# franioli/icepy4d

Measured on AMD Instinct MI355X. Metric: matched stereo image-pairs/sec (4096 kpts, 1080p), higher is better.
Workload: dtype f32

## Files before the change

icepy4d_amd/csrc/attention_bx.hip:

```cpp
#include "bf16x3.h"
#include "common.h"
#include "kernels.h"
#include "sp_post.h"

#include <cstdlib>

namespace im {

static constexpr int BKT = 32;
static constexpr int BKS = 144;
static constexpr int BVS = 192;
static constexpr int BK_PLANE = BKT * BKS, BV_PLANE = BKT * BVS;
static constexpr int B_STAGE = 3 * BK_PLANE + 3 * BV_PLANE;
static constexpr int B_LDS = 2 * B_STAGE;
static constexpr int DPL = BKT * 128;
static constexpr int D_LDS = 3 * 3 * (DPL + DPL);

__device__ __forceinline__ f32x16 mfma_attn(u32x4 a, u32x4 b, f32x16 c) {
#ifdef BX_ABL_NO_MFMA
    c[0] += __uint_as_float(a.x ^ b.x);
    return c;
#else
    return mfma_bf(a, b, c);
#endif
}

__device__ __forceinline__ void stage4(unsigned char* plane0, int plane_bytes, int off, float4 x) {
    unsigned h0, m0, l0, h1, m1, l1;
    split2(x.x, x.y, h0, m0, l0);
    split2(x.z, x.w, h1, m1, l1);
    *reinterpret_cast<u32x2*>(plane0 + off) = u32x2{h0, h1};
    *reinterpret_cast<u32x2*>(plane0 + plane_bytes + off) = u32x2{m0, m1};
    *reinterpret_cast<u32x2*>(plane0 + 2 * plane_bytes + off) = u32x2{l0, l1};
}

typedef __attribute__((address_space(3))) bf16x4 lds_bf16x4;
__device__ __forceinline__ u32x2 tr_read(const unsigned char* p) {
#ifdef BX_ABL_NO_VREAD
    const unsigned x = (unsigned)(unsigned long long)p;
    return u32x2{x, 0x3f803f80u};
#else
    const bf16x4 v = __builtin_amdgcn_ds_read_tr16_b64_v4bf16((lds_bf16x4*)(p));
    return __builtin_bit_cast(u32x2, v);
#endif
}
__device__ __forceinline__ u32x4 kf_read(const unsigned char* p) {
#ifdef BX_ABL_NO_KREAD
    const unsigned x = (unsigned)(unsigned long long)p;
    return u32x4{x, 0x3f803f80u, x, 0x3f803f80u};
#else
    return *reinterpret_cast<const u32x4*>(p);
#endif
}

static constexpr float BX_SLACK = 8.f;
__device__ __forceinline__ float bmax3(float a, float b, float c) { return __builtin_fmaxf(__builtin_fmaxf(a, b), c); }

template <bool TAIL>
__device__ __forceinline__ float softmax_ref(f32x16& s, int kb, int nk, int hh, float& m_run, float& l_run, f32x16& o0, f32x16& o1) {
    if (TAIL) {
#pragma unroll
        for (int r = 0; r < 16; ++r)
            if (kb + acc_row(r, hh) >= nk) s[r] = -INFINITY;
    }
    float mx0 = bmax3(s[0], s[1], s[2]), mx1 = bmax3(s[3], s[4], s[5]);
    mx0 = bmax3(mx0, s[6], s[7]); mx1 = bmax3(mx1, s[8], s[9]);
    mx0 = bmax3(mx0, s[10], s[11]); mx1 = bmax3(mx1, s[12], s[13]);
    float mx = bmax3(mx0, mx1, fmaxf(s[14], s[15]));
    mx = fmaxf(mx, __shfl_xor(mx, 32));
    if (__builtin_amdgcn_ballot_w64(mx > m_run + BX_SLACK) != 0) {
        asm volatile("" ::: "memory");
        const float m_new = fmaxf(m_run, mx);
        const float alpha = __builtin_amdgcn_exp2f(m_run - m_new);
        l_run *= alpha;
        o0 *= alpha;
        o1 *= alpha;
        m_run = m_new;
    }
    return (TAIL && m_run == -INFINITY) ? 0.f : m_run;
}
__device__ __forceinline__ void softmax_exp(f32x16& s, float m_use, float& l_run) {
    float r0 = 0.f, r1 = 0.f;
#pragma unroll
    for (int r = 0; r < 16; r += 2) {
        s[r] = __builtin_amdgcn_exp2f(s[r] - m_use);
        s[r + 1] = __builtin_amdgcn_exp2f(s[r + 1] - m_use);
        r0 += s[r]; r1 += s[r + 1];
    }
    float rs = r0 + r1;
    rs += __shfl_xor(rs, 32);
    l_run += rs;
}

__global__ __launch_bounds__(256) void kv_planes_kernel(AttnArgs a) {
    const long rid = (long)blockIdx.x * 32 + (threadIdx.x >> 3);
    const int d8 = threadIdx.x & 7;
    const long per_image = (long)a.heads * a.n_max;
    if (rid >= per_image * a.batch) return;
    const int z = (int)(rid / per_image), rem = (int)(rid - (long)z * per_image), head = rem / a.n_max, row = rem - head * a.n_max;
    if (a.active && a.active[(z >> 1) * a.pstride] == 0) return;
    const int n = a.n_ptr ? a.n_ptr[(z >> 1) * a.pstride + (z & 1)] : a.n_max;
    if (row >= n) return;
    const float* src = (blockIdx.y ? a.v : a.k) + (long)z * a.bstride + (long)head * a.hstride + (long)row * 64 + d8 * 8;
    const float4 u = *reinterpret_cast<const float4*>(src), w = *reinterpret_cast<const float4*>(src + 4);
    const Planes p = split8(u.x, u.y, u.z, u.w, w.x, w.y, w.z, w.w);
    unsigned char* dst = reinterpret_cast<unsigned char*>(a.planes) + ((long)blockIdx.y * per_image * a.batch + rid) * 384 + d8 * 16;
    *reinterpret_cast<u32x4*>(dst) = p.h;
    *reinterpret_cast<u32x4*>(dst + 128) = p.m;
    *reinterpret_cast<u32x4*>(dst + 256) = p.l;
}

template <bool PRE, bool DMA>
__global__ __launch_bounds__(256, 2) void flash_attn_bx_kernel(AttnArgs a) {
    static_assert(PRE || !DMA, "the DMA form stages planes");
    extern __shared__ __attribute__((aligned(16))) unsigned char bsm[];
    constexpr int RD = DMA ? 3 : 2;
    constexpr int KS = DMA ? 128 : BKS, VS = DMA ? 128 : BVS;
    constexpr int KPL = BKT * KS, VPL = BKT * VS;

    const int gsz = (a.batch % 2 == 0) ? 2 : a.batch;
    const int hz = a.heads * gsz;
    const int nqb = (a.n_max + 127) / 128;
    const int per_group = hz * nqb * (a.part ? ATTN_MAX_SPLIT : 1);
    const int grp_idx = blockIdx.x / per_group;
    const int bid = blockIdx.x - grp_idx * per_group;
    const int head = (bid % hz) % a.heads, z = grp_idx * gsz + (bid % hz) / a.heads;
    const int y = a.cross ? (z ^ 1) : z;
    if (a.active && a.active[(z >> 1) * a.pstride] == 0) return;
    const int nq = a.n_ptr ? a.n_ptr[(z >> 1) * a.pstride + (z & 1)] : a.n_max;
    const int nk_all = a.n_ptr ? a.n_ptr[(y >> 1) * a.pstride + (y & 1)] : a.n_max;
    const int qblk = (bid / hz) % nqb, split = (bid / hz) / nqb;
    const int qb = qblk * 128;
    if (qb >= nq || nk_all <= 0) return;
    int n_split = 1, k0 = 0, nk = nk_all;
    if (a.part) {
        const int steps_all = (nk_all + BKT - 1) / BKT;
        const int want = nq > 2048 ? 1 : (nq > 1024 ? 2 : ATTN_MAX_SPLIT);
        const int steps_per = (steps_all + want - 1) / want;
        n_split = (steps_all + steps_per - 1) / steps_per;
        k0 = split * steps_per * BKT;
        nk = min(nk_all - k0, steps_per * BKT);
    }
    if (split >= n_split) return;

    const int tid = threadIdx.x, lane = tid & 63, wave = tid >> 6;
    const int c = lane & 31, hh = lane >> 5;
    const int qrow = qb + wave * 32 + c;

    const float* Q = a.q + (long)z * a.bstride + (long)head * a.hstride;
    __amdgpu_buffer_rsrc_t K, V;
    u32x4 Kd = {}, Vd = {};
    if constexpr (PRE) {
        const long rows = (long)a.heads * a.n_max * a.batch;
        const unsigned char* kp = reinterpret_cast<const unsigned char*>(a.planes) + (((long)y * a.heads + head) * a.n_max + k0) * 384;
        K = make_rsrc(kp, nk * 384);
        V = make_rsrc(kp + rows * 384, nk * 384);
        if constexpr (DMA) { Kd = make_rsrc4(kp, nk * 384); Vd = make_rsrc4(kp + rows * 384, nk * 384); }
    } else {
        K = make_rsrc(a.k + (long)y * a.bstride + (long)head * a.hstride + (long)k0 * 64, nk * 256);
        V = make_rsrc(a.v + (long)y * a.bstride + (long)head * a.hstride + (long)k0 * 64, nk * 256);
    }

    u32x4 qh[4], qm[4], ql[4];
    {
        const float* qp = Q + (long)min(qrow, nq - 1) * 64 + hh * 8;
        const float c2 = a.scale * 1.4426950408889634f;
#pragma unroll
        for (int s = 0; s < 4; ++s) {
            const float4 u = *reinterpret_cast<const float4*>(qp + 16 * s), w = *reinterpret_cast<const float4*>(qp + 16 * s + 4);
            const Planes p = split8(u.x * c2, u.y * c2, u.z * c2, u.w * c2, w.x * c2, w.y * c2, w.z * c2, w.w * c2);
            qh[s] = p.h; qm[s] = p.m; ql[s] = p.l;
        }
    }

    f32x16 o0, o1;
#pragma unroll
    for (int r = 0; r < 16; ++r) { o0[r] = 0.f; o1[r] = 0.f; }
    float m_run = -INFINITY, l_run = 0.f;
    const int nt = (nk + BKT - 1) / BKT;

    unsigned char* const kring = bsm;
    unsigned char* const vring = bsm + RD * 3 * KPL;
    int kq[4], dv[2];
    const int vq = (lane & 15) >> 2;
    if constexpr (DMA) {
#pragma unroll
        for (int s4 = 0; s4 < 4; ++s4) kq[s4] = c * 128 + (((2 * s4 + hh) ^ ((c >> 1) & 7)) << 4);
        const int base = (4 * hh + vq) * 128 + (((lane >> 4) & 1) * 2 + ((lane & 3) >> 1)) * 16 + (lane & 1) * 8, sv = (vq >> 1) & 1;
        dv[0] = base + sv * 64; dv[1] = base + (1 - sv) * 64;
    } else {
#pragma unroll
        for (int s4 = 0; s4 < 4; ++s4) kq[s4] = c * BKS + hh * 16 + 32 * s4;
        const int base = (4 * hh + vq) * BVS + ((lane >> 4) & 1) * 32 + (lane & 3) * 8;
        dv[0] = base; dv[1] = base + 64;
    }

    u32x4 pk[3], pv[3];
    float4 fk[2], fv[2];
    int lk[3], lv[3];
    if constexpr (PRE) {
#pragma unroll
        for (int i = 0; i < 3; ++i) {
            const int id = tid + 256 * i, row = id / 24, rem = id - 24 * row;
            lk[i] = (rem >> 3) * BK_PLANE + row * BKS + (rem & 7) * 16;
            lv[i] = (rem >> 3) * BV_PLANE + row * BVS + (rem & 7) * 16;
        }
    }
    const unsigned voff = PRE ? tid * 16u : ((tid >> 4) * 64 + (tid & 15) * 4) * 4u;
    const int st_k = (tid >> 4) * BKS + (tid & 15) * 8, st_v = (tid >> 4) * BVS + (tid & 15) * 8;
    auto load_k = [&](int tile) {
        if constexpr (PRE) {
            const unsigned so = (unsigned)tile * (BKT * 384u);
#pragma unroll
            for (int i = 0; i < 3; ++i) pk[i] = __builtin_amdgcn_raw_buffer_load_b128(K, voff, so + 4096u * i, 0);
        } else {
            const unsigned so = (unsigned)tile * (BKT * 256u);
// ... 275 lines not shown
        if (threadIdx.x == 0) {
            unsigned long long* cp = a.clock + 2 * (blockIdx.x % CLOCK_PROBE_SLOTS);
            cp[0] = ck1 - ck0; cp[1] = cr1 - cr0;
        }
    }
    {
        const int t = nt - 1;
        m_use = softmax_ref<true>(sc, t * BKT, nk, hh, m_run, l_run, o0, o1);
        softmax_exp(sc, m_use, l_run);
        pv_mul(r0, sc);
    }

    if (n_split > 1) {
        const long prow = (((long)z * a.heads + head) * a.n_max + min(qrow, a.n_max - 1)) * 66;
        const long pstride = (long)a.batch * a.heads * a.n_max * 66;
        float* pp = a.part + (long)split * pstride + prow;
        if (qrow < nq) {
#pragma unroll
            for (int g = 0; g < 4; ++g) {
                *reinterpret_cast<float2*>(pp + 8 * g + 4 * hh) = make_float2(o0[4 * g], o0[4 * g + 1]);
                *reinterpret_cast<float2*>(pp + 8 * g + 4 * hh + 2) = make_float2(o0[4 * g + 2], o0[4 * g + 3]);
                *reinterpret_cast<float2*>(pp + 32 + 8 * g + 4 * hh) = make_float2(o1[4 * g], o1[4 * g + 1]);
                *reinterpret_cast<float2*>(pp + 32 + 8 * g + 4 * hh + 2) = make_float2(o1[4 * g + 2], o1[4 * g + 3]);
            }
            if (hh == 0) { pp[64] = m_run; pp[65] = l_run; }
        }
        __threadfence();
        __syncthreads();
        int* flag = reinterpret_cast<int*>(bsm);
        if (tid == 0) {
            int* cnt = a.counters + ((long)z * a.heads + head) * nqb + qblk;
            const int old = atomicAdd(cnt, 1);
            *flag = (old == n_split - 1);
            if (old == n_split - 1) *cnt = 0;
        }
        __syncthreads();
        if (!*flag) return;
        __threadfence();
        float m = -INFINITY;
        for (int sidx = 0; sidx < n_split; ++sidx) m = fmaxf(m, a.part[(long)sidx * pstride + prow + 64]);
        l_run = 0.f;
#pragma unroll
        for (int r = 0; r < 16; ++r) { o0[r] = 0.f; o1[r] = 0.f; }
        for (int sidx = 0; sidx < n_split; ++sidx) {
            const float* ps = a.part + (long)sidx * pstride + prow;
            const float w = __builtin_amdgcn_exp2f(ps[64] - m);
            l_run += w * ps[65];
#pragma unroll
            for (int g = 0; g < 4; ++g)
#pragma unroll
                for (int q = 0; q < 4; ++q) {
                    o0[4 * g + q] += w * ps[8 * g + 4 * hh + q];
                    o1[4 * g + q] += w * ps[32 + 8 * g + 4 * hh + q];
                }
        }
    }

    if (qrow < nq) {
        const float inv = 1.f / l_run;
        float* op = a.out + (long)z * a.out_bstride + (long)qrow * a.ldo + head * 64;
#pragma unroll
        for (int g = 0; g < 4; ++g) {
            const float4 w0 = make_float4(o0[4 * g] * inv, o0[4 * g + 1] * inv, o0[4 * g + 2] * inv, o0[4 * g + 3] * inv);
            const float4 w1 = make_float4(o1[4 * g] * inv, o1[4 * g + 1] * inv, o1[4 * g + 2] * inv, o1[4 * g + 3] * inv);
            *reinterpret_cast<float4*>(op + 8 * g + 4 * hh) = w0;
            *reinterpret_cast<float4*>(op + 32 + 8 * g + 4 * hh) = w1;
        }
    }
}

hipError_t launch_attn_planes(const AttnArgs& a, hipStream_t s) {
    static const bool f32_form = [] { const char* e = getenv("IM_ATTN_F32"); return e && atoi(e) != 0; }();
    if (!a.planes || a.n_max <= 0 || f32_form || a.f32_form) return hipSuccess;
    const long rows = (long)a.batch * a.heads * a.n_max;
    hipLaunchKernelGGL(kv_planes_kernel, dim3((unsigned)((rows + 31) / 32), 2), dim3(256), 0, s, a);
    return hipGetLastError();
}

hipError_t launch_flash_attn_bx(const AttnArgs& a, hipStream_t s) {
    static size_t lds_pre[IM_MAX_DEVICES] = {0}, lds_cut[IM_MAX_DEVICES] = {0};
    dim3 grid(((a.n_max + 127) / 128) * a.heads * a.batch * (a.part ? ATTN_MAX_SPLIT : 1)), block(256);
    static size_t lds_dma[IM_MAX_DEVICES] = {0};
    static const bool reg_staging = [] { const char* e = getenv("IM_ATTN_REG_STAGING"); return e && atoi(e) != 0; }();
    if (a.planes && !reg_staging) {
        if (hipError_t e = ensure_dyn_lds(reinterpret_cast<const void*>(&flash_attn_bx_kernel<true, true>), D_LDS, lds_dma); e != hipSuccess) return e;
        hipLaunchKernelGGL((flash_attn_bx_kernel<true, true>), grid, block, D_LDS, s, a);
    } else if (a.planes) {
        if (hipError_t e = ensure_dyn_lds(reinterpret_cast<const void*>(&flash_attn_bx_kernel<true, false>), B_LDS, lds_pre); e != hipSuccess) return e;
        hipLaunchKernelGGL((flash_attn_bx_kernel<true, false>), grid, block, B_LDS, s, a);
    } else {
        if (hipError_t e = ensure_dyn_lds(reinterpret_cast<const void*>(&flash_attn_bx_kernel<false, false>), B_LDS, lds_cut); e != hipSuccess) return e;
        hipLaunchKernelGGL((flash_attn_bx_kernel<false, false>), grid, block, B_LDS, s, a);
    }
    return hipGetLastError();
}

}
```

icepy4d_amd/csrc/capi.hip:

```cpp
#include "ctx.h"

#include <cstdio>
#include <cstdlib>
#include <cstring>

using namespace im;

extern "C" {

int im_version(void) { return 100; }

int im_ctx_create(int device, im_ctx** out) {
    if (!out) return -1;
    int ndev = 0;
    if (hipGetDeviceCount(&ndev) != hipSuccess || device < 0 || device >= ndev) return -2;
    if (hipSetDevice(device) != hipSuccess) return -3;
    im_ctx* c = new im_ctx();
    c->device = device;
    const char* g = getenv("IM_DEBUG_GUARDS");
    c->guards_on = g && g[0] == '1';
    *out = c;
    return 0;
}

// ... 13 lines not shown
    g.A = d_a; g.lda = k; g.W = d_w; g.ldw = k; g.bias = d_bias; g.N = n; g.K = k; g.m_max = m;
    g.C = d_c; g.ldc = n; g.alpha = alpha; g.epi = EPI_BIAS; g.big_tile = big_tile & 1; g.bx = (big_tile >> 1) & 1;
    IM_HIP(ctx, launch_gemm(g, (hipStream_t)stream));
    return 0;
}

int im_ffn_fused(im_ctx* ctx, int act, float* d_x, const float* d_att, const float* h_w0, const float* h_b0, const float* h_ln_g,
                   const float* h_ln_b, const float* h_w3, const float* h_b3, int n_images, int n_rows, const int32_t* d_n, void* stream) {
    IM_CHECK_CTX(ctx);
    if (n_images < 1 || n_rows < 1 || act < 0 || act > 1 || (act == 0 && (!h_ln_g || !h_ln_b))) return ctx->fail(-12, "im_ffn_fused: bad arguments");
    if (act == 1) h_ln_g = h_ln_b = h_b0;
    const std::vector<float> p0 = pack_frag_weights(h_w0, 512, 512), p3 = pack_frag_weights(h_w3, 256, 512);
    const size_t sizes[6] = {p0.size(), 512, 512, 512, p3.size(), 256};
    const float* src[6] = {p0.data(), h_b0, h_ln_g, h_ln_b, p3.data(), h_b3};
    float* d[6] = {nullptr, nullptr, nullptr, nullptr, nullptr, nullptr};
    hipError_t e = hipSuccess;
    for (int i = 0; i < 6 && e == hipSuccess; ++i) {
        e = hipMalloc(&d[i], sizes[i] * sizeof(float));
        if (e == hipSuccess) e = hipMemcpy(d[i], src[i], sizes[i] * sizeof(float), hipMemcpyHostToDevice);
    }
    hipStream_t st = (hipStream_t)stream;
    if (e == hipSuccess) {
        FfnArgs f;
        f.act = act; f.x = d_x; f.x_bstride = (long)n_rows * 256; f.att = d_att; f.att_bstride = (long)n_rows * 256;
        f.w0p = d[0]; f.b0 = d[1]; f.ln_g = d[2]; f.ln_b = d[3]; f.w3p = d[4]; f.b3 = d[5];
        f.m_max = n_rows; f.batch = n_images; f.m_ptr = d_n; f.pstride = 2;
        e = ctx->timed("ffn_fused", st, [&] { return launch_ffn_fused(f, st); });
    }
    const hipError_t e2 = hipStreamSynchronize(st);
    for (int i = 0; i < 6; ++i) hipFree(d[i]);
    IM_HIP(ctx, e);
    IM_HIP(ctx, e2);
    return 0;
}

static int conv3x3_entry(im_ctx* ctx, bool wino, const float* d_in, const float* h_weight, const float* h_bias, float* d_out,
                         int b, int h, int w, int cin, int cout, int relu, int pool, void* stream);

int im_conv3x3(im_ctx* ctx, const float* d_in, const float* h_weight, const float* h_bias, float* d_out, int b, int h,
               int w, int cin, int cout, int relu, int pool, void* stream) {
    return conv3x3_entry(ctx, false, d_in, h_weight, h_bias, d_out, b, h, w, cin, cout, relu, pool, stream);
}

int im_conv3x3_winograd(im_ctx* ctx, const float* d_in, const float* h_weight, const float* h_bias, float* d_out, int b,
                        int h, int w, int cin, int cout, int relu, int pool, void* stream) {
    return conv3x3_entry(ctx, true, d_in, h_weight, h_bias, d_out, b, h, w, cin, cout, relu, pool, stream);
}

static int conv3x3_entry(im_ctx* ctx, bool wino, const float* d_in, const float* h_weight, const float* h_bias, float* d_out,
                         int b, int h, int w, int cin, int cout, int relu, int pool, void* stream) {
    IM_CHECK_CTX(ctx);
    if (cin % 16 || cout % 64) return ctx->fail(-10, "im_conv3x3: cin %% 16 and cout %% 64 must be 0");
    std::vector<float> packed = wino ? pack_conv3x3_wino(h_weight, cout, cin) : pack_conv3x3(h_weight, cout, cin);
    std::vector<float> planes = wino ? pack_conv3x3_wino_bx(h_weight, cout, cin) : std::vector<float>(1);
    const size_t sizes[3] = {packed.size(), (size_t)cout, planes.size()};
    const float* src[3] = {packed.data(), h_bias, planes.data()};
    float* d[3] = {nullptr, nullptr, nullptr};
    hipError_t e = hipSuccess;
    for (int i = 0; i < 3 && e == hipSuccess; ++i) {
        e = hipMalloc(&d[i], sizes[i] * sizeof(float));
        if (e == hipSuccess) e = hipMemcpy(d[i], src[i], sizes[i] * sizeof(float), hipMemcpyHostToDevice);
    }
    hipStream_t st = (hipStream_t)stream;
    if (e == hipSuccess) {
        ConvArgs a;
        a.in = d_in; a.w = d[0]; a.bias = d[1]; a.out = d_out; a.B = b; a.H = h; a.W = w; a.Cin = cin; a.Cout = cout;
        a.relu = relu; a.pool = pool;
        if (wino) a.wx = d[2];
        e = ctx->timed(wino ? "conv_wino" : "conv_direct", st, [&] { return wino ? launch_conv3x3_wino(a, st) : launch_conv3x3(a, st); });
    }
    const hipError_t e2 = hipStreamSynchronize(st);
    for (int i = 0; i < 3; ++i) hipFree(d[i]);
    IM_HIP(ctx, e);
    IM_HIP(ctx, e2);
    return 0;
}

int im_flash_attn(im_ctx* ctx, const float* d_q, const float* d_k, const float* d_v, float* d_out, const int32_t* d_n,
                  int n_max, int batch, int heads, int cross, float scale, void* stream) {
    IM_CHECK_CTX(ctx);
    AttnArgs a;
    a.q = d_q; a.k = d_k; a.v = d_v; a.hstride = (long)n_max * 64; a.bstride = a.hstride * heads;
    a.out = d_out; a.ldo = heads * 64; a.out_bstride = (long)n_max * a.ldo;
    a.n_ptr = d_n; a.n_max = n_max; a.batch = batch; a.heads = heads; a.cross = cross & 1; a.f32_form = (cross >> 1) & 1; a.scale = scale;
    im_ctx::StageScratch& sc = ctx->scratch;
    const bool wants_planes = !(cross & 4) && !a.f32_form;
    IM_GROW(ctx, ctx->grow(sc.attn_part, attn_part_floats(n_max, batch, heads) * sizeof(float), "stage_attn_part"), -11, "im_flash_attn: out of device memory");
    IM_GROW(ctx, ctx->grow(sc.attn_cnt, attn_counter_ints(n_max, batch, heads) * sizeof(int), "stage_attn_cnt", true), -11, "im_flash_attn: out of device memory");
    if (wants_planes) IM_GROW(ctx, ctx->grow(sc.attn_planes, attn_planes_bytes(n_max, batch, heads), "stage_attn_planes"), -11, "im_flash_attn: out of device memory");
    a.part = sc.attn_part.as<float>(); a.counters = sc.attn_cnt.as<int>(); a.planes = wants_planes ? sc.attn_planes.as<unsigned char>() : nullptr;
    IM_HIP(ctx, launch_attn_planes(a, (hipStream_t)stream));
    IM_HIP(ctx, launch_flash_attn(a, (hipStream_t)stream));
    IM_GUARD_CHECK(ctx, (hipStream_t)stream, "im_flash_attn");
    return 0;
}

}
```

icepy4d_amd/csrc/kernels.h:

```cpp
#pragma once
#include <hip/hip_runtime.h>
#include <stdint.h>
#include <vector>

namespace im {

enum GemmEpi {
    EPI_BIAS = 0,
    EPI_BIAS_RESID = 1,
    EPI_HEADS = 2,
    EPI_QKV_ROPE = 3,
    EPI_BIAS_RELU = 4,
    EPI_HEADS_QV = 5,
};

struct GemmArgs {
    const float* A = nullptr;  long a_bstride = 0;  int lda = 0;
    const float* A1 = nullptr; long a1_bstride = 0; int lda1 = 0; int ksplit = 0;
    const float* W = nullptr;  int ldw = 0; long w_bstride = 0;
    const float* bias = nullptr;
    const int* sel = nullptr; long w_sel_stride = 0; long bias_sel_stride = 0;
    int N = 0, K = 0;
    int m_max = 0;
    const int* m_ptr = nullptr;
    const int* n_ptr = nullptr;
    const int* active = nullptr;
    int pstride = 2;
    int pair_batched = 0;
    int batch = 1;
    float alpha = 1.f;
    float* C = nullptr; long c_bstride = 0; int ldc = 0;
    const float* R = nullptr; long r_bstride = 0; int ldr = 0;
    float* q = nullptr; float* k = nullptr; float* v = nullptr; long head_bstride = 0; long head_stride = 0;
    const float* cs = nullptr; const float* sn = nullptr; long enc_bstride = 0;
    int epi = EPI_BIAS;
    int big_tile = 0;
    int bx = 0;
    const void* wp = nullptr;
};
hipError_t launch_gemm(const GemmArgs& a, hipStream_t s);
hipError_t launch_proj_rows(const GemmArgs& a, hipStream_t s);

struct FfnArgs {
    int act = 0;
    float* x = nullptr; long x_bstride = 0;
    const float* att = nullptr; long att_bstride = 0;
    const float* w0p = nullptr; const float* b0 = nullptr;
    const float* ln_g = nullptr; const float* ln_b = nullptr;
    const float* w3p = nullptr; const float* b3 = nullptr;
    int m_max = 0; int batch = 1;
    const int* m_ptr = nullptr;
    const int* active = nullptr;
    int pstride = 2;
};
hipError_t launch_ffn_fused(const FfnArgs& a, hipStream_t s);
std::vector<float> pack_frag_weights(const float* w, int n, int k);

struct AttnArgs {
    const float* q = nullptr; const float* k = nullptr; const float* v = nullptr;
    long bstride = 0; long hstride = 0;
    float* out = nullptr; long out_bstride = 0; int ldo = 256;
    const int* n_ptr = nullptr;
    int pstride = 2;
    int n_max = 0; int batch = 2; int heads = 4; int cross = 0;
    float scale = 1.f;
    const int* active = nullptr;
    float* part = nullptr;
    int* counters = nullptr;
    void* planes = nullptr;
    int f32_form = 0;
    unsigned long long* clock = nullptr;
};
static constexpr int CLOCK_PROBE_SLOTS = 4096;
static constexpr int ATTN_MAX_SPLIT = 4;
inline size_t attn_part_floats(int n_max, int batch, int heads) { return (size_t)ATTN_MAX_SPLIT * batch * heads * n_max * 66; }
inline size_t attn_planes_bytes(int n_max, int batch, int heads) { return (size_t)2 * batch * heads * n_max * 384; }
inline size_t attn_counter_ints(int n_max, int batch, int heads) { return (size_t)batch * heads * ((n_max + 127) / 128); }
hipError_t launch_flash_attn(const AttnArgs& a, hipStream_t s);
hipError_t launch_attn_planes(const AttnArgs& a, hipStream_t s);
hipError_t launch_flash_attn_bx(const AttnArgs& a, hipStream_t s);

struct ConvArgs {
    const float* in = nullptr;
    const float* w = nullptr;
    const float* bias = nullptr;
    float* out = nullptr;
    int B = 1, H = 0, W = 0, Cin = 0, Cout = 0;
    int pool = 0;
    int relu = 1;
    const uint8_t* img = nullptr;
    int img_channels = 1;
    int gray_mode = 0;
    const float* w1 = nullptr;
    const float* b1 = nullptr;
    const float* w1q = nullptr;
    const void* wx = nullptr;
    int f32_form = 0;
    unsigned long long* clock = nullptr;
};
hipError_t launch_conv3x3(const ConvArgs& a, hipStream_t s);
hipError_t launch_conv3x3_wino(const ConvArgs& a, hipStream_t s);
hipError_t launch_conv3x3_wino_bx2(const ConvArgs& a, hipStream_t s);
hipError_t launch_conv1a(const uint8_t* img, int channels, int gray_mode, const float* w, const float* bias, float* out, int B, int H,
                         int W, hipStream_t s);

}
```

Measured before the change: 175.2.

## Add two-tile flash attention kernel for wide query blocks sharing K/V staging

Adds a new attention kernel in which each wave handles two 32-row query tiles (256 queries per block), so every K/V tile staged into LDS and read into registers feeds twice as many MFMAs. When nq exceeds 2048, the original kernel exits early for those images and the new kernel is launched afterwards. Shared softmax and MFMA helpers move into a header. The aim is to halve LDS and DMA traffic per unit of work, at the cost of higher register pressure (launch bounds 256,1), fewer blocks and an extra launch.

```diff
diff --git a/icepy4d_amd/csrc/attention_bx.h b/icepy4d_amd/csrc/attention_bx.h
--- /dev/null
+++ b/icepy4d_amd/csrc/attention_bx.h
@@ -0,0 +1,79 @@
+#pragma once
+#include "bf16x3.h"
+#include "common.h"
+#include "kernels.h"
+
+namespace im {
+
+static constexpr int BKT = 32;
+static constexpr int DPL = BKT * 128;
+static constexpr int D_LDS = 3 * 3 * (DPL + DPL);
+
+__device__ __forceinline__ f32x16 mfma_attn(u32x4 a, u32x4 b, f32x16 c) {
+#ifdef BX_ABL_NO_MFMA
+    c[0] += __uint_as_float(a.x ^ b.x);
+    return c;
+#else
+    return mfma_bf(a, b, c);
+#endif
+}
+
+typedef __attribute__((address_space(3))) bf16x4 lds_bf16x4;
+__device__ __forceinline__ u32x2 tr_read(const unsigned char* p) {
+#ifdef BX_ABL_NO_VREAD
+    const unsigned x = (unsigned)(unsigned long long)p;
+    return u32x2{x, 0x3f803f80u};
+#else
+    const bf16x4 v = __builtin_amdgcn_ds_read_tr16_b64_v4bf16((lds_bf16x4*)(p));
+    return __builtin_bit_cast(u32x2, v);
+#endif
+}
+__device__ __forceinline__ u32x4 kf_read(const unsigned char* p) {
+#ifdef BX_ABL_NO_KREAD
+    const unsigned x = (unsigned)(unsigned long long)p;
+    return u32x4{x, 0x3f803f80u, x, 0x3f803f80u};
+#else
+    return *reinterpret_cast<const u32x4*>(p);
+#endif
+}
+
+static constexpr float BX_SLACK = 8.f;
+__device__ __forceinline__ float bmax3(float a, float b, float c) { return __builtin_fmaxf(__builtin_fmaxf(a, b), c); }
+
+template <bool TAIL>
+__device__ __forceinline__ float softmax_ref(f32x16& s, int kb, int nk, int hh, float& m_run, float& l_run, f32x16& o0, f32x16& o1) {
+    if (TAIL) {
+#pragma unroll
+        for (int r = 0; r < 16; ++r)
+            if (kb + acc_row(r, hh) >= nk) s[r] = -INFINITY;
+    }
+    float mx0 = bmax3(s[0], s[1], s[2]), mx1 = bmax3(s[3], s[4], s[5]);
+    mx0 = bmax3(mx0, s[6], s[7]); mx1 = bmax3(mx1, s[8], s[9]);
+    mx0 = bmax3(mx0, s[10], s[11]); mx1 = bmax3(mx1, s[12], s[13]);
+    float mx = bmax3(mx0, mx1, fmaxf(s[14], s[15]));
+    mx = fmaxf(mx, __shfl_xor(mx, 32));
+    if (__builtin_amdgcn_ballot_w64(mx > m_run + BX_SLACK) != 0) {
+        asm volatile("" ::: "memory");
+        const float m_new = fmaxf(m_run, mx);
+        const float alpha = __builtin_amdgcn_exp2f(m_run - m_new);
+        l_run *= alpha;
+        o0 *= alpha;
+        o1 *= alpha;
+        m_run = m_new;
+    }
+    return (TAIL && m_run == -INFINITY) ? 0.f : m_run;
+}
+__device__ __forceinline__ void softmax_exp(f32x16& s, float m_use, float& l_run) {
+    float r0 = 0.f, r1 = 0.f;
+#pragma unroll
+    for (int r = 0; r < 16; r += 2) {
+        s[r] = __builtin_amdgcn_exp2f(s[r] - m_use);
+        s[r + 1] = __builtin_amdgcn_exp2f(s[r + 1] - m_use);
+        r0 += s[r]; r1 += s[r + 1];
+    }
+    float rs = r0 + r1;
+    rs += __shfl_xor(rs, 32);
+    l_run += rs;
+}
+
+}
diff --git a/icepy4d_amd/csrc/attention_bx.hip b/icepy4d_amd/csrc/attention_bx.hip
--- a/icepy4d_amd/csrc/attention_bx.hip
+++ b/icepy4d_amd/csrc/attention_bx.hip
@@ -1,29 +1,15 @@
-#include "bf16x3.h"
-#include "common.h"
-#include "kernels.h"
+#include "attention_bx.h"
 #include "sp_post.h"
 
 #include <cstdlib>
 
 namespace im {
 
-static constexpr int BKT = 32;
 static constexpr int BKS = 144;
 static constexpr int BVS = 192;
 static constexpr int BK_PLANE = BKT * BKS, BV_PLANE = BKT * BVS;
 static constexpr int B_STAGE = 3 * BK_PLANE + 3 * BV_PLANE;
 static constexpr int B_LDS = 2 * B_STAGE;
-static constexpr int DPL = BKT * 128;
-static constexpr int D_LDS = 3 * 3 * (DPL + DPL);
-
-__device__ __forceinline__ f32x16 mfma_attn(u32x4 a, u32x4 b, f32x16 c) {
-#ifdef BX_ABL_NO_MFMA
-    c[0] += __uint_as_float(a.x ^ b.x);
-    return c;
-#else
-    return mfma_bf(a, b, c);
-#endif
-}
 
 __device__ __forceinline__ void stage4(unsigned char* plane0, int plane_bytes, int off, float4 x) {
     unsigned h0, m0, l0, h1, m1, l1;
@@ -32,64 +18,6 @@
     *reinterpret_cast<u32x2*>(plane0 + off) = u32x2{h0, h1};
     *reinterpret_cast<u32x2*>(plane0 + plane_bytes + off) = u32x2{m0, m1};
     *reinterpret_cast<u32x2*>(plane0 + 2 * plane_bytes + off) = u32x2{l0, l1};
-}
-
-typedef __attribute__((address_space(3))) bf16x4 lds_bf16x4;
-__device__ __forceinline__ u32x2 tr_read(const unsigned char* p) {
-#ifdef BX_ABL_NO_VREAD
-    const unsigned x = (unsigned)(unsigned long long)p;
-    return u32x2{x, 0x3f803f80u};
-#else
-    const bf16x4 v = __builtin_amdgcn_ds_read_tr16_b64_v4bf16((lds_bf16x4*)(p));
-    return __builtin_bit_cast(u32x2, v);
-#endif
-}
-__device__ __forceinline__ u32x4 kf_read(const unsigned char* p) {
-#ifdef BX_ABL_NO_KREAD
-    const unsigned x = (unsigned)(unsigned long long)p;
-    return u32x4{x, 0x3f803f80u, x, 0x3f803f80u};
-#else
-    return *reinterpret_cast<const u32x4*>(p);
-#endif
-}
-
-static constexpr float BX_SLACK = 8.f;
-__device__ __forceinline__ float bmax3(float a, float b, float c) { return __builtin_fmaxf(__builtin_fmaxf(a, b), c); }
-
-template <bool TAIL>
-__device__ __forceinline__ float softmax_ref(f32x16& s, int kb, int nk, int hh, float& m_run, float& l_run, f32x16& o0, f32x16& o1) {
-    if (TAIL) {
-#pragma unroll
-        for (int r = 0; r < 16; ++r)
-            if (kb + acc_row(r, hh) >= nk) s[r] = -INFINITY;
-    }
-    float mx0 = bmax3(s[0], s[1], s[2]), mx1 = bmax3(s[3], s[4], s[5]);
-    mx0 = bmax3(mx0, s[6], s[7]); mx1 = bmax3(mx1, s[8], s[9]);
-    mx0 = bmax3(mx0, s[10], s[11]); mx1 = bmax3(mx1, s[12], s[13]);
-    float mx = bmax3(mx0, mx1, fmaxf(s[14], s[15]));
-    mx = fmaxf(mx, __shfl_xor(mx, 32));
-    if (__builtin_amdgcn_ballot_w64(mx > m_run + BX_SLACK) != 0) {
-        asm volatile("" ::: "memory");
-        const float m_new = fmaxf(m_run, mx);
-        const float alpha = __builtin_amdgcn_exp2f(m_run - m_new);
-        l_run *= alpha;
-        o0 *= alpha;
-        o1 *= alpha;
-        m_run = m_new;
-    }
-    return (TAIL && m_run == -INFINITY) ? 0.f : m_run;
-}
-__device__ __forceinline__ void softmax_exp(f32x16& s, float m_use, float& l_run) {
-    float r0 = 0.f, r1 = 0.f;
-#pragma unroll
-    for (int r = 0; r < 16; r += 2) {
-        s[r] = __builtin_amdgcn_exp2f(s[r] - m_use);
-        s[r + 1] = __builtin_amdgcn_exp2f(s[r + 1] - m_use);
-        r0 += s[r]; r1 += s[r + 1];
-    }
-    float rs = r0 + r1;
-    rs += __shfl_xor(rs, 32);
-    l_run += rs;
 }
 
 __global__ __launch_bounds__(256) void kv_planes_kernel(AttnArgs a) {
@@ -132,6 +60,7 @@
     const int qblk = (bid / hz) % nqb, split = (bid / hz) / nqb;
     const int qb = qblk * 128;
     if (qb >= nq || nk_all <= 0) return;
+    if (a.wide_elsewhere && nq > ATTN_WIDE_Q) return;
     int n_split = 1, k0 = 0, nk = nk_all;
     if (a.part) {
         const int steps_all = (nk_all + BKT - 1) / BKT;
@@ -573,9 +502,23 @@
     dim3 grid(((a.n_max + 127) / 128) * a.heads * a.batch * (a.part ? ATTN_MAX_SPLIT : 1)), block(256);
     static size_t lds_dma[IM_MAX_DEVICES] = {0};
     static const bool reg_staging = [] { const char* e = getenv("IM_ATTN_REG_STAGING"); return e && atoi(e) != 0; }();
+    static const bool two_tiles = [] { const char* e = getenv("IM_ATTN_TWO_TILES"); return !e || atoi(e) != 0; }();
     if (a.planes && !reg_staging) {
+        static int cus[IM_MAX_DEVICES] = {0};
+        int dev = 0;
+        if (hipError_t e = hipGetDevice(&dev); e != hipSuccess) return e;
+        dev = dev < IM_MAX_DEVICES ? dev : 0;
+        if (cus[dev] == 0 && hipDeviceGetAttribute(&cus[dev], hipDeviceAttributeMultiprocessorCount, dev) != hipSuccess) cus[dev] = 256;
+        const long blocks2 = (long)((a.n_max + 255) / 256) * a.heads * a.batch;
+        const long rounds = (blocks2 + cus[dev] - 1) / cus[dev];
+        AttnArgs b = a;
+        b.wide_elsewhere = two_tiles && !a.one_tile && a.n_max > ATTN_WIDE_Q && (a.any_width || (rounds * cus[dev] - blocks2) * 32 <= rounds * cus[dev]);
         if (hipError_t e = ensure_dyn_lds(reinterpret_cast<const void*>(&flash_attn_bx_kernel<true, true>), D_LDS, lds_dma); e != hipSuccess) return e;
-        hipLaunchKernelGGL((flash_attn_bx_kernel<true, true>), grid, block, D_LDS, s, a);
+        hipLaunchKernelGGL((flash_attn_bx_kernel<true, true>), grid, block, D_LDS, s, b);
+        if (b.wide_elsewhere) {
+            if (hipError_t e = hipGetLastError(); e != hipSuccess) return e;
+            return launch_flash_attn_bx2(b, s);
+        }
     } else if (a.planes) {
         if (hipError_t e = ensure_dyn_lds(reinterpret_cast<const void*>(&flash_attn_bx_kernel<true, false>), B_LDS, lds_pre); e != hipSuccess) return e;
         hipLaunchKernelGGL((flash_attn_bx_kernel<true, false>), grid, block, B_LDS, s, a);
diff --git a/icepy4d_amd/csrc/attention_bx2.hip b/icepy4d_amd/csrc/attention_bx2.hip
--- /dev/null
+++ b/icepy4d_amd/csrc/attention_bx2.hip
@@ -0,0 +1,363 @@
+#include "attention_bx.h"
+#include "sp_post.h"
+
+namespace im {
+
+__global__ __launch_bounds__(256, 1) void flash_attn_bx2_kernel(AttnArgs a) {
+    extern __shared__ __attribute__((aligned(16))) unsigned char bsm[];
+    constexpr int KPL = DPL, VPL = DPL, VS = 128;
+
+    const int gsz = (a.batch % 2 == 0) ? 2 : a.batch;
+    const int hz = a.heads * gsz;
+    const int nqb = (a.n_max + 255) / 256;
+    const int per_group = hz * nqb;
+    const int grp_idx = blockIdx.x / per_group;
+    const int bid = blockIdx.x - grp_idx * per_group;
+    const int head = (bid % hz) % a.heads, z = grp_idx * gsz + (bid % hz) / a.heads;
+    const int y = a.cross ? (z ^ 1) : z;
+    if (a.active && a.active[(z >> 1) * a.pstride] == 0) return;
+    const int nq = a.n_ptr ? a.n_ptr[(z >> 1) * a.pstride + (z & 1)] : a.n_max;
+    const int nk = a.n_ptr ? a.n_ptr[(y >> 1) * a.pstride + (y & 1)] : a.n_max;
+    const int qb = (bid / hz) * 256;
+    if (nq <= ATTN_WIDE_Q || qb >= nq || nk <= 0) return;
+
+    const int tid = threadIdx.x, lane = tid & 63, wave = tid >> 6;
+    const int c = lane & 31, hh = lane >> 5;
+    const int qrow[2] = {qb + wave * 64 + c, qb + wave * 64 + 32 + c};
+
+    const float* Q = a.q + (long)z * a.bstride + (long)head * a.hstride;
+    const long rows = (long)a.heads * a.n_max * a.batch;
+    const unsigned char* kpl = reinterpret_cast<const unsigned char*>(a.planes) + ((long)y * a.heads + head) * a.n_max * 384;
+    const u32x4 Kd = make_rsrc4(kpl, nk * 384), Vd = make_rsrc4(kpl + rows * 384, nk * 384);
+
+    u32x4 qh[2][4], qm[2][4], ql[2][4];
+    {
+        const float c2 = a.scale * 1.4426950408889634f;
+#pragma unroll
+        for (int T = 0; T < 2; ++T) {
+            const float* qp = Q + (long)min(qrow[T], nq - 1) * 64 + hh * 8;
+#pragma unroll
+            for (int s = 0; s < 4; ++s) {
+                const float4 u = *reinterpret_cast<const float4*>(qp + 16 * s), w = *reinterpret_cast<const float4*>(qp + 16 * s + 4);
+                const Planes p = split8(u.x * c2, u.y * c2, u.z * c2, u.w * c2, w.x * c2, w.y * c2, w.z * c2, w.w * c2);
+                qh[T][s] = p.h; qm[T][s] = p.m; ql[T][s] = p.l;
+            }
+        }
+    }
+
+    f32x16 o0[2], o1[2];
+#pragma unroll
+    for (int T = 0; T < 2; ++T)
+#pragma unroll
+        for (int r = 0; r < 16; ++r) { o0[T][r] = 0.f; o1[T][r] = 0.f; }
+#define BX_ACC(x) asm volatile("" : "+a"(x))
+#pragma unroll
+    for (int T = 0; T < 2; ++T) {
+#pragma unroll
+        for (int s = 0; s < 4; ++s) { BX_ACC(qh[T][s]); BX_ACC(qm[T][s]); BX_ACC(ql[T][s]); }
+    }
+    float m_run[2] = {-INFINITY, -INFINITY}, l_run[2] = {0.f, 0.f};
+    const int nt = (nk + BKT - 1) / BKT;
+
+    unsigned char* const kring = bsm;
+    unsigned char* const vring = bsm + 3 * 3 * KPL;
+    int kq[4], dv[2];
+    const int vq = (lane & 15) >> 2;
+#pragma unroll
+    for (int s4 = 0; s4 < 4; ++s4) kq[s4] = c * 128 + (((2 * s4 + hh) ^ ((c >> 1) & 7)) << 4);
+    {
+        const int base = (4 * hh + vq) * 128 + (((lane >> 4) & 1) * 2 + ((lane & 3) >> 1)) * 16 + (lane & 1) * 8, sv = (vq >> 1) & 1;
+        dv[0] = base + sv * 64; dv[1] = base + (1 - sv) * 64;
+    }
+    const int drow = 8 * wave + (lane >> 3), dpc = lane & 7;
+    const unsigned dvoff_k = drow * 384u + ((dpc ^ ((drow >> 1) & 7)) << 4), dvoff_v = drow * 384u + ((dpc ^ (((drow >> 1) & 1) << 2)) << 4);
+    const unsigned wave_u = __builtin_amdgcn_readfirstlane(tid >> 6);
+    const unsigned lds_k = __builtin_amdgcn_readfirstlane((unsigned)(unsigned long)(lds_ptr_t)kring) + wave_u * 1024u;
+    const unsigned lds_v = __builtin_amdgcn_readfirstlane((unsigned)(unsigned long)(lds_ptr_t)vring) + wave_u * 1024u;
+    auto dma_k1 = [&](int tile, int stage, int i) {
+        dma16(Kd, __builtin_amdgcn_readfirstlane(lds_k + (unsigned)stage * (3u * DPL) + i * DPL), dvoff_k, __builtin_amdgcn_readfirstlane((unsigned)tile * (BKT * 384u) + i * 128u));
+    };
+    auto dma_v1 = [&](int tile, int stage, int i) {
+        dma16(Vd, __builtin_amdgcn_readfirstlane(lds_v + (unsigned)stage * (3u * DPL) + i * DPL), dvoff_v, __builtin_amdgcn_readfirstlane((unsigned)tile * (BKT * 384u) + i * 128u));
+    };
+    auto dma_k = [&](int tile, int stage) {
+#pragma unroll
+        for (int i = 0; i < 3; ++i) dma_k1(tile, stage, i);
+    };
+    auto dma_v = [&](int tile, int stage) {
+#pragma unroll
+        for (int i = 0; i < 3; ++i) dma_v1(tile, stage, i);
+    };
+    auto qk = [&](int stage, f32x16 (&out)[2]) {
+        const unsigned char* const kp = kring + stage * 3 * KPL;
+        f32x16 xa[2], xb[2];
+#pragma unroll
+        for (int T = 0; T < 2; ++T)
+#pragma unroll
+            for (int r = 0; r < 16; ++r) { xa[T][r] = 0.f; xb[T][r] = 0.f; }
+#pragma unroll
+        for (int s = 0; s < 4; ++s) {
+            const u32x4 kh = kf_read(kp + kq[s]), km = kf_read(kp + KPL + kq[s]), kl = kf_read(kp + 2 * KPL + kq[s]);
+#pragma unroll
+            for (int T = 0; T < 2; ++T) {
+                f32x16& x = (s & 1) ? xb[T] : xa[T];
+                x = mfma_attn(kh, ql[T][s], x);
+                x = mfma_attn(kl, qh[T][s], x);
+                x = mfma_attn(km, qm[T][s], x);
+                x = mfma_attn(kh, qm[T][s], x);
+                x = mfma_attn(km, qh[T][s], x);
+                x = mfma_attn(kh, qh[T][s], x);
+            }
+        }
+#pragma unroll
+        for (int T = 0; T < 2; ++T) out[T] = xa[T] + xb[T];
+    };
+    auto pv_mul = [&](int stage, const f32x16 (&p)[2]) {
+        const unsigned char* const vp = vring + stage * 3 * VPL;
+#pragma unroll
+        for (int s = 0; s < 2; ++s) {
+            Planes pp[2];
+#pragma unroll
+            for (int T = 0; T < 2; ++T)
+                pp[T] = split8(p[T][8 * s + 0], p[T][8 * s + 1], p[T][8 * s + 2], p[T][8 * s + 3], p[T][8 * s + 4], p[T][8 * s + 5], p[T][8 * s + 6], p[T][8 * s + 7]);
+#pragma unroll
+            for (int dt = 0; dt < 2; ++dt) {
+                const unsigned char* vb = vp + (16 * s) * VS + dv[dt];
+                const u32x2 h0 = tr_read(vb), h1 = tr_read(vb + 8 * VS);
+                const u32x2 m0 = tr_read(vb + VPL), m1 = tr_read(vb + VPL + 8 * VS);
+                const u32x2 l0 = tr_read(vb + 2 * VPL), l1 = tr_read(vb + 2 * VPL + 8 * VS);
+                const u32x4 vh = {h0.x, h0.y, h1.x, h1.y}, vm = {m0.x, m0.y, m1.x, m1.y}, vl = {l0.x, l0.y, l1.x, l1.y};
+#pragma unroll
+                for (int T = 0; T < 2; ++T) {
+                    f32x16& o = dt ? o1[T] : o0[T];
+                    o = mfma_attn(vh, pp[T].l, o);
+                    o = mfma_attn(vl, pp[T].h, o);
+                    o = mfma_attn(vm, pp[T].m, o);
+                    o = mfma_attn(vh, pp[T].m, o);
+                    o = mfma_attn(vm, pp[T].h, o);
+                    o = mfma_attn(vh, pp[T].h, o);
+                }
+            }
+        }
+    };
+
+    f32x16 sc[2], sn[2];
+    dma_k(0, 0); dma_k(1, 1); dma_v(0, 0);
+    asm volatile("s_waitcnt vmcnt(0)" ::: "memory");
+    __syncthreads();
+    dma_k(2, 2); dma_v(1, 1);
+    qk(0, sc);
+    __syncthreads();
+
+    static constexpr int PA[6] = {0, 2, 1, 0, 1, 0}, PB[6] = {2, 0, 1, 1, 0, 0};
+    float m_use[2] = {0.f, 0.f};
+    if (nt >= 2) {
+#pragma unroll
+        for (int T = 0; T < 2; ++T) m_use[T] = softmax_ref<false>(sc[T], 0, nk, hh, m_run[T], l_run[T], o0[T], o1[T]);
+    }
+    int r0 = 0, r1 = 1, r2 = 2;
+    unsigned long long ck0 = 0, cr0 = 0;
+    if (a.clock) { ck0 = __builtin_amdgcn_s_memtime(); cr0 = __builtin_amdgcn_s_memrealtime(); }
+    u32x4 kf[2][3];
+#pragma unroll
+    for (int pl = 0; pl < 3; ++pl) kf[0][pl] = kf_read(kring + 3 * KPL + pl * KPL + kq[0]);
+    for (int t = 0; t < nt - 2; ++t) {
+        const unsigned char* const kp = kring + r1 * 3 * KPL;
+        const unsigned char* const vp = vring + r0 * 3 * VPL;
+        u32x2 vr[2][6];
+        __builtin_amdgcn_sched_barrier(0);
+
+        float ra[2][8], rb[2][8], rsum0[2] = {0.f, 0.f}, rsum1[2] = {0.f, 0.f};
+        unsigned ch[2][8], cm[2][8], cl[2][8];
+#define BX_PIN(x) asm volatile("" : "+v"(x))
+        auto expo = [&](int T, int r) {
+#ifdef BX_ABL_NO_EXPCUT
+            return;
+#endif
+            float x = sc[T][r];
+            BX_PIN(x);
+            x = __builtin_amdgcn_exp2f(x - m_use[T]);
+            BX_PIN(x);
+            sc[T][r] = x;
+            if (r & 1) rsum1[T] += x; else rsum0[T] += x;
+        };
+        auto cut_a = [&](int T, int i) {
+#ifdef BX_ABL_NO_EXPCUT
+            ch[T][i] = __float_as_uint(sc[T][2 * i]); cm[T][i] = __float_as_uint(sc[T][2 * i + 1]); cl[T][i] = ch[T][i]; return;
+#endif
+            float x = sc[T][2 * i], y2 = sc[T][2 * i + 1];
+            BX_PIN(x); BX_PIN(y2);
+            ch[T][i] = cvt_pk(x, y2);
+            ra[T][i] = x - __uint_as_float(ch[T][i] << 16);
+            rb[T][i] = y2 - __uint_as_float(ch[T][i] & 0xffff0000u);
+            BX_PIN(ra[T][i]); BX_PIN(rb[T][i]);
+        };
+        auto cut_b = [&](int T, int i) {
+#ifdef BX_ABL_NO_EXPCUT
+            return;
+#endif
+            BX_PIN(ra[T][i]); BX_PIN(rb[T][i]);
+            cm[T][i] = cvt_pk(ra[T][i], rb[T][i]);
+            ra[T][i] -= __uint_as_float(cm[T][i] << 16);
+            rb[T][i] -= __uint_as_float(cm[T][i] & 0xffff0000u);
+            BX_PIN(ra[T][i]); BX_PIN(rb[T][i]);
+        };
+        auto cut_l = [&](int T, int i) {
+#ifdef BX_ABL_NO_EXPCUT
+            return;
+#endif
+            BX_PIN(ra[T][i]);
+            cl[T][i] = cvt_pk(ra[T][i], rb[T][i]);
+            BX_PIN(cl[T][i]);
+        };
+
+        f32x16 xa[2], xb[2];
+#pragma unroll
+        for (int T = 0; T < 2; ++T)
+#pragma unroll
+            for (int r = 0; r < 16; ++r) { xa[T][r] = 0.f; xb[T][r] = 0.f; }
+#pragma unroll
+        for (int s4 = 0; s4 < 4; ++s4) {
+#pragma unroll
+            for (int T = 0; T < 2; ++T) {
+#pragma unroll
+                for (int j = 0; j < 6; ++j) {
+                    const int v = 6 * s4 + j;
+                    const u32x4 qp = PB[j] == 0 ? qh[T][s4] : (PB[j] == 1 ? qm[T][s4] : ql[T][s4]);
+                    if (j & 1) xb[T] = mfma_attn(kf[s4 & 1][PA[j]], qp, xb[T]);
+                    else xa[T] = mfma_attn(kf[s4 & 1][PA[j]], qp, xa[T]);
+                    if (v < 8) expo(T, v);
+                    else if (v < 16) { if (v & 1) cut_b(T, (v - 8) >> 1); else cut_a(T, (v - 8) >> 1); }
+                    else { expo(T, v - 8); if (v < 20) cut_l(T, v - 16); }
+                    if (s4 < 3 && T == 0 && j >= 1 && j <= 3) kf[(s4 + 1) & 1][j - 1] = kf_read(kp + (j - 1) * KPL + kq[s4 + 1]);
+                    if (s4 == 3 && T == 0) vr[0][j] = tr_read(vp + dv[0] + (j >> 1) * VPL + (j & 1) * 8 * VS);
+                    __builtin_amdgcn_sched_barrier(0);
+                }
+            }
+        }
+        asm volatile("s_waitcnt vmcnt(0)" ::: "memory");
+#ifndef BX_ABL_NO_BARRIER
+        __syncthreads();
+#endif
+        __builtin_amdgcn_sched_barrier(0);
+        float mxn[2] = {0.f, 0.f}, mxs[2] = {0.f, 0.f};
+#pragma unroll
+        for (int g = 0; g < 4; ++g) {
+            const int ks = g >> 1;
+            const u32x4 vf[3] = {u32x4{vr[g & 1][0].x, vr[g & 1][0].y, vr[g & 1][1].x, vr[g & 1][1].y},
+                                 u32x4{vr[g & 1][2].x, vr[g & 1][2].y, vr[g & 1][3].x, vr[g & 1][3].y},
+                                 u32x4{vr[g & 1][4].x, vr[g & 1][4].y, vr[g & 1][5].x, vr[g & 1][5].y}};
+#pragma unroll
+            for (int T = 0; T < 2; ++T) {
+                const u32x4 pp[3] = {u32x4{ch[T][4 * ks], ch[T][4 * ks + 1], ch[T][4 * ks + 2], ch[T][4 * ks + 3]},
+                                     u32x4{cm[T][4 * ks], cm[T][4 * ks + 1], cm[T][4 * ks + 2], cm[T][4 * ks + 3]},
+                                     u32x4{cl[T][4 * ks], cl[T][4 * ks + 1], cl[T][4 * ks + 2], cl[T][4 * ks + 3]}};
+#pragma unroll
+                for (int j = 0; j < 6; ++j) {
+                    const int v = 6 * g + j;
+                    if (g & 1) o1[T] = mfma_attn(vf[PA[j]], pp[PB[j]], o1[T]);
+                    else o0[T] = mfma_attn(vf[PA[j]], pp[PB[j]], o0[T]);
+                    if (v < 8) { if (v & 1) cut_b(T, 4 + (v >> 1)); else cut_a(T, 4 + (v >> 1)); }
+                    else if (v < 12) cut_l(T, 4 + v - 8);
+                    if (v >= 8 && v < 16) {
+                        float u0 = xa[T][2 * (v - 8)] + xb[T][2 * (v - 8)], u1 = xa[T][2 * (v - 8) + 1] + xb[T][2 * (v - 8) + 1];
+                        BX_PIN(u0); BX_PIN(u1);
+                        sn[T][2 * (v - 8)] = u0; sn[T][2 * (v - 8) + 1] = u1;
+                    }
+                    if (v == 12) {
+                        float rs = rsum0[T] + rsum1[T];
+                        rs += __shfl_xor(rs, 32);
+                        l_run[T] += rs;
+                    }
+                    if (v >= 9 && v <= 16) {
+                        const int i = v - 9;
+                        float u = i == 0 ? bmax3(sn[T][0], sn[T][1], sn[T][2]) : (i == 7 ? fmaxf(mxn[T], sn[T][15]) : bmax3(mxn[T], sn[T][2 * i + 1], sn[T][2 * i + 2]));
+                        BX_PIN(u);
+                        mxn[T] = u;
+                    }
+                    if (v == 19) mxs[T] = __shfl_xor(mxn[T], 32);
+#ifndef BX_ABL_NO_STAGE
+                    if (g == 1 && (j & 1)) {
+                        if (T == 0) dma_k1(t + 3, r0, j >> 1);
+                        else dma_v1(t + 2, r2, j >> 1);
+                    }
+#endif
+                    if (g == 3 && T == 1 && !(j & 1)) kf[0][j >> 1] = kf_read(kring + r2 * 3 * KPL + (j >> 1) * KPL + kq[0]);
+                    if (g < 3 && T == 0) {
+                        const int gn = g + 1;
+                        vr[gn & 1][j] = tr_read(vp + (16 * (gn >> 1)) * VS + dv[gn & 1] + (j >> 1) * VPL + (j & 1) * 8 * VS);
+                    }
+                    __builtin_amdgcn_sched_barrier(0);
+                }
+            }
+        }
+#pragma unroll
+        for (int T = 0; T < 2; ++T) mxn[T] = fmaxf(mxn[T], mxs[T]);
+#pragma unroll
+        for (int T = 0; T < 2; ++T) {
+            if (__builtin_amdgcn_ballot_w64(mxn[T] > m_run[T] + BX_SLACK) != 0) {
+                asm volatile("" ::: "memory");
+                const float m_new = fmaxf(m_run[T], mxn[T]);
+                const float alpha = __builtin_amdgcn_exp2f(m_run[T] - m_new);
+                l_run[T] *= alpha;
+                o0[T] *= alpha;
+                o1[T] *= alpha;
+                m_run[T] = m_new;
+            }
+            m_use[T] = m_run[T];
+            sc[T] = sn[T];
+        }
+        { const int rr = r0; r0 = r1; r1 = r2; r2 = rr; }
+    }
+#undef BX_PIN
+#undef BX_ACC
+    asm volatile("s_waitcnt vmcnt(0)" ::: "memory");
+    if (nt >= 2) {
+        __syncthreads();
+        qk(r1, sn);
+#pragma unroll
+        for (int T = 0; T < 2; ++T) softmax_exp(sc[T], m_use[T], l_run[T]);
+        pv_mul(r0, sc);
+#pragma unroll
+        for (int T = 0; T < 2; ++T) sc[T] = sn[T];
+        { const int rr = r0; r0 = r1; r1 = r2; r2 = rr; }
+        __syncthreads();
+    }
+    if (a.clock && nt > 8) {
+        const unsigned long long ck1 = __builtin_amdgcn_s_memtime(), cr1 = __builtin_amdgcn_s_memrealtime();
+        if (threadIdx.x == 0) {
+            unsigned long long* cp = a.clock + 2 * (blockIdx.x % CLOCK_PROBE_SLOTS);
+            cp[0] = ck1 - ck0; cp[1] = cr1 - cr0;
+        }
+    }
+#pragma unroll
+    for (int T = 0; T < 2; ++T) {
+        m_use[T] = softmax_ref<true>(sc[T], (nt - 1) * BKT, nk, hh, m_run[T], l_run[T], o0[T], o1[T]);
+        softmax_exp(sc[T], m_use[T], l_run[T]);
+    }
+    pv_mul(r0, sc);
+
+#pragma unroll
+    for (int T = 0; T < 2; ++T) {
+        if (qrow[T] >= nq) continue;
+        const float inv = 1.f / l_run[T];
+        float* op = a.out + (long)z * a.out_bstride + (long)qrow[T] * a.ldo + head * 64;
+#pragma unroll
+        for (int g = 0; g < 4; ++g) {
+            const float4 w0 = make_float4(o0[T][4 * g] * inv, o0[T][4 * g + 1] * inv, o0[T][4 * g + 2] * inv, o0[T][4 * g + 3] * inv);
+            const float4 w1 = make_float4(o1[T][4 * g] * inv, o1[T][4 * g + 1] * inv, o1[T][4 * g + 2] * inv, o1[T][4 * g + 3] * inv);
+            *reinterpret_cast<float4*>(op + 8 * g + 4 * hh) = w0;
+            *reinterpret_cast<float4*>(op + 32 + 8 * g + 4 * hh) = w1;
+        }
+    }
+}
+
+hipError_t launch_flash_attn_bx2(const AttnArgs& a, hipStream_t s) {
+    static size_t lds_dma[IM_MAX_DEVICES] = {0};
+    if (!a.planes) return hipErrorInvalidValue;
+    if (hipError_t e = ensure_dyn_lds(reinterpret_cast<const void*>(&flash_attn_bx2_kernel), D_LDS, lds_dma); e != hipSuccess) return e;
+    hipLaunchKernelGGL(flash_attn_bx2_kernel, dim3(((a.n_max + 255) / 256) * a.heads * a.batch), dim3(256), D_LDS, s, a);
+    return hipGetLastError();
+}
+
+}
diff --git a/icepy4d_amd/csrc/capi.hip b/icepy4d_amd/csrc/capi.hip
--- a/icepy4d_amd/csrc/capi.hip
+++ b/icepy4d_amd/csrc/capi.hip
@@ -119,7 +119,7 @@
     AttnArgs a;
     a.q = d_q; a.k = d_k; a.v = d_v; a.hstride = (long)n_max * 64; a.bstride = a.hstride * heads;
     a.out = d_out; a.ldo = heads * 64; a.out_bstride = (long)n_max * a.ldo;
-    a.n_ptr = d_n; a.n_max = n_max; a.batch = batch; a.heads = heads; a.cross = cross & 1; a.f32_form = (cross >> 1) & 1; a.scale = scale;
+    a.n_ptr = d_n; a.n_max = n_max; a.batch = batch; a.heads = heads; a.cross = cross & 1; a.f32_form = (cross >> 1) & 1; a.one_tile = (cross >> 3) & 1; a.any_width = 1; a.scale = scale;
     im_ctx::StageScratch& sc = ctx->scratch;
     const bool wants_planes = !(cross & 4) && !a.f32_form;
     IM_GROW(ctx, ctx->grow(sc.attn_part, attn_part_floats(n_max, batch, heads) * sizeof(float), "stage_attn_part"), -11, "im_flash_attn: out of device memory");
diff --git a/icepy4d_amd/csrc/kernels.h b/icepy4d_amd/csrc/kernels.h
--- a/icepy4d_amd/csrc/kernels.h
+++ b/icepy4d_amd/csrc/kernels.h
@@ -68,17 +68,20 @@
     float* part = nullptr;
     int* counters = nullptr;
     void* planes = nullptr;
+    int one_tile = 0; int any_width = 0; int wide_elsewhere = 0;
     int f32_form = 0;
     unsigned long long* clock = nullptr;
 };
 static constexpr int CLOCK_PROBE_SLOTS = 4096;
 static constexpr int ATTN_MAX_SPLIT = 4;
+static constexpr int ATTN_WIDE_Q = 2048;
 inline size_t attn_part_floats(int n_max, int batch, int heads) { return (size_t)ATTN_MAX_SPLIT * batch * heads * n_max * 66; }
 inline size_t attn_planes_bytes(int n_max, int batch, int heads) { return (size_t)2 * batch * heads * n_max * 384; }
 inline size_t attn_counter_ints(int n_max, int batch, int heads) { return (size_t)batch * heads * ((n_max + 127) / 128); }
 hipError_t launch_flash_attn(const AttnArgs& a, hipStream_t s);
 hipError_t launch_attn_planes(const AttnArgs& a, hipStream_t s);
 hipError_t launch_flash_attn_bx(const AttnArgs& a, hipStream_t s);
+hipError_t launch_flash_attn_bx2(const AttnArgs& a, hipStream_t s);
 
 struct ConvArgs {
     const float* in = nullptr;
```

Result: no change. 176.6 (median of 6 runs) (+0.8%).
